# ai-forever/Kandinsky-5

Measured on AMD Instinct MI355X. Metric: DiT denoising steps/sec (2B Lite, 5s 768x512 latent), higher is better.
Workload: dtype bf16

## Files before the change

include/k5.h:

```cpp
#ifndef K5_H
#define K5_H
#include <stdint.h>
#ifdef __cplusplus
extern "C" {
#endif

typedef enum {
  K5_OK = 0, K5_ERR_ARG = 1, K5_ERR_ALIGN = 2, K5_ERR_HIP = 3, K5_ERR_STATE = 4, K5_ERR_KEY = 5,
  K5_ERR_UNSUPPORTED = 6
} k5_status;
typedef enum { K5_F32 = 0, K5_BF16 = 1, K5_F16 = 2 } k5_dtype;
typedef enum { K5_EPI_BIAS = 0, K5_EPI_BIAS_M = 1, K5_EPI_GELU = 2, K5_EPI_GATE = 3, K5_EPI_F32 = 4  } k5_epilogue;

#define K5_ABI_VERSION 11
int k5_abi_version(void);
const char* k5_last_error(void);


int k5_gemm_bf16(const void* A, const void* W, const float* bias, void* C, int M, int N, int K, int lda,
                 int ldw, int ldc, int epilogue, const void* resid, int ldr, const float* gate, void* stream);
int k5_gemm_bf16_variant(const void* A, const void* W, const float* bias, void* C, int M, int N, int K, int lda, int ldw, int ldc,
                         int epilogue, const void* resid, int ldr, const float* gate, void* stream, int kernel, int token_tile);

int k5_gemm_bf16_f32out(const void* A, const void* W, float* C, int M, int N, int K, int lda, int ldw, int ldc,
// ... 37 lines not shown
                                          float* state, int flags, int late_pass, void* workspace, void* stream);
int k5_attention_bf16_prescaled_qnorm_pass(const void* Q, const void* Kc, const void* Vt, void* O, int H, int q_len, int kv_len, int ldq,
                                           int ldk, int ldvt, int ldo, const float* q_norm_w, const float* q_cos, const float* q_sin,
                                           int* head_flags, const float* kmax, int tile_off0, int tile_cnt, float* state, int flags,
                                           int late_pass, void* workspace, void* stream);
int k5_attention_bf16_prescaled_auto(const void* Q, const void* Kc, const void* Vt, void* O, int H, int q_len, int kv_len,
                                     int ldq, int ldk, int ldvt, int ldo, const int* head_flags, int variant, void* workspace,
                                     void* stream);
int64_t k5_attention_balance_size(int H, int q_len);
int k5_attention_bf16_balanced(const void* Q, const void* K, const void* Vt, void* O, int H, int q_len, int kv_len,
                               int ldq, int ldk, int ldvt, int ldo, float score_bound, void* workspace, void* stream);

int64_t k5_nabla_workspace_size(int H, int num_blocks);
int k5_nabla_select_bf16(const void* q, const void* k, int ldq, int ldk, int H, int N, int T, int Hb, int Wb, int wT,
                         int wH, int wW, float P, void* workspace, void* stream);
int k5_attention_nabla_bf16(const void* Q, const void* K, const void* Vt, void* O, int H, int N, int ldq, int ldk,
                            int ldvt, int ldo, float score_bound, const void* workspace, void* stream);
int k5_nabla_mask_u8(const void* workspace, int H, int num_blocks, void* out_u8, void* stream);
int k5_nabla_select_rect_bf16(const void* q, const void* k, int ldq, int ldk, int H, int Nq, int q_block0, int N, int T,
                              int Hb, int Wb, int wT, int wH, int wW, float P, void* workspace, void* stream);
int k5_attention_nabla_rect_bf16(const void* Q, const void* K, const void* Vt, void* O, int H, int Nq, int N, int ldq,
                                 int ldk, int ldvt, int ldo, float score_bound, const void* workspace, int vt_chunk_keys,
                                 int64_t vt_chunk_stride, void* stream);
int k5_nabla_select_rect_local_bf16(const void* q, const void* k, int ldq, int ldk, int H, int Nq, int q_block0, int N, int T, int Hb,
                                    int Wb, int wT, int wH, int wW, float P, void* workspace, int local_block0, int local_blocks,
                                    void* stream);
int k5_attention_nabla_rect_prescaled_pass(const void* Q, const void* Kc, const void* Vt, void* O, int H, int Nq, int N, int ldq, int ldk,
                                           int ldvt, int ldo, const void* workspace, int vt_chunk_keys, int64_t vt_chunk_stride,
                                           int* head_flags, const float* kmax, int pass, float* state, void* stream);
int k5_nabla_mask_rect_u8(const void* workspace, int H, int q_blocks, int num_blocks, void* out_u8, void* stream);

int k5_attention_bf16_bounded(const void* Q, const void* K, const void* Vt, void* O, int H, int q_len,
                              int kv_len, int ldq, int ldk, int ldvt, int ldo, float score_bound, void* stream);

int k5_ln_modulate_bf16(const void* x, const float* scale, const float* shift, void* out, int rows, int D,
                        int ldx, int ldo, void* stream);
int k5_rmsnorm_rope_bf16(void* x, const float* weight, const float* cos_tab, const float* sin_tab, int rows,
                         int H, int ld, int heads_per_weight, int rope_heads, void* stream);
int k5_rmsnorm_rope_stats_bf16(void* x, const float* weight, const float* cos_tab, const float* sin_tab, int rows, int H,
                               int ld, int heads_per_weight, int rope_heads, float out_scale, int scale_from_head,
                               float* stats, void* stream);
int k5_gate_sum_bf16(const void* x, const void* y, const float* gate, void* out, int rows, int D, void* stream);
int k5_magcache_stats_bf16(const void* vis, const void* ori, const void* prev, void* res, double* sums, int rows, int D, void* stream);
int k5_gemv_f32(const float* x, const float* W, const float* b, float* y, int N, int K, int silu_in,
                const float* add, void* stream);
int k5_time_features_f32(float t, float* out, int D, void* stream);
int k5_ln_affine_bf16(const void* x, const float* w, const float* b, void* out_bf16, float* out_f32, int rows,
                      int D, void* stream);
int k5_rope_table_f32(float* cos_tab, float* sin_tab, const int32_t* pos_t, const int32_t* pos_h,
                      const int32_t* pos_w, int T, int H, int W, int n0, int n1, int n2, float s0, float s1,
                      float s2, const int32_t* tok_perm, void* stream);
int k5_patchify_bf16(const float* x, void* out, int T, int H, int W, int x_channels, int Cin_total, int Kpad,
                     const int32_t* tok_perm, void* stream);
int k5_patchify_cond_bf16(const float* x, const float* vcond, void* out, int T, int H, int W, int x_channels, int Cin_total,
                          int Kpad, const int32_t* tok_perm, void* stream);
int k5_unpatchify_bf16(const void* x, void* out, int T, int Hp, int Wp, int C, int ldx,
                       const int32_t* tok_perm, void* stream);
int k5_cfg_euler(float* img, const void* v_cond, const void* v_uncond, float w, float dt, int64_t n,
                 void* stream);

typedef struct k5_dit k5_dit;

typedef struct k5_dit_config {
  int in_visual_dim, in_text_dim, in_text_dim2, time_dim, out_visual_dim;
  int patch_size[3];
  int model_dim, ff_dim, num_text_blocks, num_visual_blocks;
// ... 139 lines not shown
```

kandinsky-5_amd/csrc/attn_fwd.hip:

```cpp
#include <stdlib.h>

#include <type_traits>
#include "k5_common.h"
#include "k5_kernels.h"

namespace {

constexpr int QB = 256;
constexpr int KB = 64;
constexpr int TILE = 64 * 128;

constexpr float K5_ATTN_EXP_LIMIT = 90.f;
constexpr float K5_ATTN_ROW_MIN = 3.2311743e-27f;
constexpr float K5_ATTN_ROWOFF_LIMIT = 190.f;
constexpr float K5_ATTN_ANCHOR_ADD = 20.f, K5_ATTN_ANCHOR_SPREAD = 1.4f, K5_ATTN_ANCHOR_EXTRA_MAX = 60.f;
inline float anchor_spread(int kv_total) {
  const float c = sqrtf(2.f * logf(512.f));
  return K5_ATTN_ANCHOR_SPREAD * (sqrtf(2.f * logf((float)(kv_total > 512 ? kv_total : 512))) - c) / c;
}
constexpr float K5_ATTN_ROW_MAX = 5.1922969e33f;
constexpr int K5_ANCHOR_TILES = 32;
#ifndef K5_ATTN_WAVE_ROWS_DEFAULT
#define K5_ATTN_WAVE_ROWS_DEFAULT 32
#endif
#ifndef K5_ATTN_PAIR
#define K5_ATTN_PAIR 1
#endif

struct AttnP {
  const bf16_t* Q; const bf16_t* K; const bf16_t* Vt; bf16_t* O;
  int H, q_len, kv_len, ldq, ldk, ldvt, ldo, nqb;
  float c;
  const int* sp_begin;
  const int* head_flags; int my_flag;
// ... 621 lines not shown
        float* st_o = state_o(qt); float* st_ml = state_ml(qt, g);
#pragma unroll
        for (int dt = 0; dt < 4; ++dt) *reinterpret_cast<f32x4*>(st_o + 256 * dt) = ot[dt][qt];
        st_ml[0] = BOUNDED ? 0.f : (fresh ? -1e30f : -nm[qt][0]);
        st_ml[1] = g == 0 ? lt[qt][0] : 0.f;
        if (BOUNDED && PRE && p.kmax && nm[qt][0] != 0.f && !((lt[qt][0] >= K5_ATTN_ROW_MIN || (anchored && !SPARSE)) && lt[qt][0] < K5_ATTN_ROW_MAX) && seen) {
          if (p.job_flags) const_cast<int*>(p.job_flags)[lid] = p.late_pass ? 2 : 1;
          else const_cast<int*>(p.head_flags)[h] = p.late_pass ? 2 : 0;
        }
      }
    return;
  }

#pragma unroll
  for (int qt = 0; qt < QT; ++qt) {
    const float l_tot = lt[qt][0];
    const float inv = l_tot > 0.f ? 1.0f / l_tot : 0.f;
    const int q = q0 + 16 * qt + l15;
    if (BOUNDED && PRE && p.kmax && q < p.q_len && nm[qt][0] != 0.f && !(l_tot >= K5_ATTN_ROW_MIN && l_tot < K5_ATTN_ROW_MAX)) {
      if (p.job_flags) const_cast<int*>(p.job_flags)[lid] = p.late_pass ? 2 : 1;
      else const_cast<int*>(p.head_flags)[h] = p.late_pass ? 2 : 0;
    }
    if (q < p.q_len) {
      bf16_t* op = p.O + (size_t)q * p.ldo + h * 64 + 4 * g;
#pragma unroll
      for (int dt = 0; dt < 4; ++dt) {
        u32x2 o = {pack_bf16x2(ot[dt][qt][0] * inv, ot[dt][qt][1] * inv), pack_bf16x2(ot[dt][qt][2] * inv, ot[dt][qt][3] * inv)};
        *reinterpret_cast<u32x2*>(op + 16 * dt) = o;
      }
    }
  }
}

template <bool BOUNDED, bool SPARSE, bool RANGE>
__global__ __launch_bounds__(512, 4) void attn_fwd32_kernel(AttnP p) {
  __shared__ __attribute__((aligned(16))) char smem[4 * TILE];
  char* sK = smem;
  char* sV = smem + 2 * TILE;
  const int tid = threadIdx.x, lane = tid & 63, wave = tid >> 6, hi = lane >> 5, l31 = lane & 31;
  const int gid = xcd_remap(blockIdx.x, gridDim.x);
  const int part = RANGE ? gid % p.splits : 0;
  const int lid = p.job0 + (RANGE ? gid / p.splits : gid);
  const int h = lid / p.nqb, qb = lid % p.nqb;
  const int q0 = qb * QB + wave * 32;

  bf16x8 qf[4];
  {
    const bf16_t* qp = p.Q + (size_t)min(q0 + l31, p.q_len - 1) * p.ldq + h * 64 + 8 * hi;
#pragma unroll
    for (int kk = 0; kk < 4; ++kk) qf[kk] = *reinterpret_cast<const bf16x8*>(qp + 16 * kk);
  }
  const int lrow = tid >> 3, lc = tid & 7;
  const bf16_t* kbase = p.K + h * 64 + 8 * lc;
  const bf16_t* vbase = p.Vt + (size_t)(h * 64 + lrow) * p.ldvt + 8 * lc;
  const int lds_off = lds_swz(lrow, lc);
  const int* sp_list = SPARSE ? p.sp_list + (size_t)(h * p.nqb + qb) * p.sp_stride : nullptr;
  const int Tall = SPARSE ? p.sp_cnt[h * p.nqb + qb] : p.tile_cnt;
  const int E0 = RANGE ? (int)(((long long)Tall * part) / p.splits) : 0;
  const int T = RANGE ? (int)(((long long)Tall * (part + 1)) / p.splits) : Tall;
  const int nfull = p.kv_len / KB;
  auto tile_of = [&](int e) -> int {
    if (SPARSE) return sp_list[e] & 0xffffff;
    if (!RANGE) return e;
    if (p.seg_len > 0) {
      int si = e / p.seg_len;
      const int j = e - si * p.seg_len;
// ... 313 lines not shown
      }
      const float extra = fminf(fmaxf(spread * (m - sm * inv_n), 0.f), K5_ATTN_ANCHOR_EXTRA_MAX);
      const int row = 64 * blk + 16 * qt + l15;
      if (g == 0 && row < q_len) out[(size_t)h * q_len + row] = ceilf(m + extra) + K5_ATTN_ANCHOR_ADD;
    }
  }
}

}


size_t k5_attention_state_bytes(int H, int q_len) { return (size_t)H * ((q_len + QB - 1) / QB) * QB * (64 + 8) * sizeof(float); }

constexpr int K5_ATTN_MAX_SPLITS = 6;
size_t k5_attention_balance_bytes(int H, int q_len) {
  return (size_t)K5_ATTN_MAX_SPLITS * k5_attention_state_bytes(H, q_len) + (size_t)H * ((q_len + 63) / 64 + 1) * sizeof(int);
}
namespace {
inline int* attn_job_flags(float* ws, int H, int q_len) { return reinterpret_cast<int*>(reinterpret_cast<char*>(ws) + (size_t)K5_ATTN_MAX_SPLITS * k5_attention_state_bytes(H, q_len)); }
inline size_t attn_job_flags_bytes(int H, int q_len) { return (size_t)H * ((q_len + 63) / 64 + 1) * sizeof(int); }
}

namespace {
int g_attn_slots = 0;
int attn_slots() {
  if (!g_attn_slots) {
    int dev = 0; hipDeviceProp_t prop;
    if (hipGetDevice(&dev) != hipSuccess || hipGetDeviceProperties(&prop, dev) != hipSuccess) return 512;
    g_attn_slots = 2 * (prop.multiProcessorCount > 0 ? prop.multiProcessorCount : 256);
  }
  static const bool pipe = getenv("K5_ATTN_WAVE_ROWS") && atoi(getenv("K5_ATTN_WAVE_ROWS")) > 100;
  return pipe ? g_attn_slots / 2 : g_attn_slots;
}
}

int k5_launch_attn_pref_update(float* balance_ws, int H, int q_len, int group_rows, int* prefer_online, hipStream_t stream, unsigned int* leave_sig) {
  if (!balance_ws || !prefer_online || H <= 0 || q_len <= 0) return K5_ERR_ARG;
  const int nqb = (q_len + 64 * group_rows - 1) / (64 * group_rows);
  hipLaunchKernelGGL(attn_pref_update_kernel, dim3(H), dim3(64), 0, stream, attn_job_flags(balance_ws, H, q_len), nqb, H, prefer_online, leave_sig);
  return hipGetLastError() == hipSuccess ? K5_OK : K5_ERR_HIP;
}

int k5_launch_attn_flags(float* qstat, float* kstat, int nk, int kstride, int H, int force_online, int* flags,
                         unsigned long long* counters, hipStream_t stream, float* kmax_out, const int* prefer_online, float* rstat, float* krad_out,
                         int nq, int qstride, bool anchored, unsigned int* leave_sig) {
  if ((rstat == nullptr) != (krad_out == nullptr) || (rstat && !kmax_out) || nq < 1) return K5_ERR_ARG;
  if (!qstat || !kstat || !flags || H <= 0 || nk <= 0) return K5_ERR_ARG;
  hipLaunchKernelGGL(attn_flags_kernel, dim3((H + 63) / 64), dim3(64), 0, stream, qstat, kstat, nk, kstride, H,
                     kmax_out ? K5_ATTN_ROWOFF_LIMIT : K5_ATTN_EXP_LIMIT, force_online, flags, counters, kmax_out, kmax_out ? prefer_online : nullptr,
                     rstat, krad_out, nq, qstride, anchored ? 1 : 0, leave_sig);
  return hipGetLastError() == hipSuccess ? K5_OK : K5_ERR_HIP;
}

int k5_launch_attn_row_anchor(const void* Q, const void* Kc, int H, int q_len, int kv_len, int ldq, int ldk, int key0, int kv_total,
                              const float* kmax, float* out, hipStream_t stream) {
  if (!Q || !Kc || !kmax || !out || H <= 0 || q_len <= 0 || kv_len < KB || (kv_len % KB) || (ldq & 7) || (ldk & 7)) return K5_ERR_ARG;
  hipLaunchKernelGGL(attn_row_anchor_kernel, dim3((q_len + 1023) / 1024, H), dim3(512), 0, stream, (const bf16_t*)Q, (const bf16_t*)Kc, q_len, kv_len,
                     ldq, ldk, key0, anchor_spread(kv_total > kv_len ? kv_total : kv_len), kmax, out);
  return hipGetLastError() == hipSuccess ? K5_OK : K5_ERR_HIP;
}

int k5_launch_attention_bf16_range(const void* Q, const void* K, const void* Vt, void* O, int H, int q_len,
                                   int kv_len, int ldq, int ldk, int ldvt, int ldo, float score_bound,
                                   int vt_chunk_keys, long long vt_chunk_stride, int tile_off0, int tile_cnt, int tile_skip_at,
                                   int tile_skip_n, float* state, int flags, hipStream_t stream, float* ws, bool k_prescaled,
                                   const int* head_flags, int variant, const K5TileSegments* seg, const float* kmax, int late_pass,
                                   const K5QueryNorm* qn, const K5KeyCentre* kc) {
// ... 20 lines not shown
  }
  p.q_norm_w = qn ? qn->w : nullptr; p.q_cos = qn ? qn->cos : nullptr; p.q_sin = qn ? qn->sin : nullptr;
  p.variant_counters = qn ? qn->counters : nullptr;
  if (p.q_norm_w) {
    if (k_prescaled) {
      if (!p.q_cos || !p.q_sin || (kmax && !head_flags)) return K5_ERR_ARG;
    } else if (!(score_bound > 0.f && score_bound * p.c <= K5_ATTN_EXP_LIMIT)) {
      return K5_ERR_UNSUPPORTED;
    }
  }
  p.vt_chunk_keys = vt_chunk_keys; p.vt_chunk_stride = vt_chunk_stride;
  const dim3 block(512);
  const bool bounded = score_bound > 0.f && score_bound * p.c <= K5_ATTN_EXP_LIMIT;
  p.sp_list = nullptr; p.sp_cnt = nullptr; p.sp_stride = 0;
  const int total_tiles = (kv_len + KB - 1) / KB;
  if (tile_cnt < 0) tile_cnt = total_tiles - tile_off0;
  p.seg_len = 0; p.seg_stride = 0; p.seg_skip = 0x7fffffff;
  if (seg && seg->len > 0) {
    if (tile_off0 < 0 || tile_cnt <= 0 || seg->stride < seg->len || seg->skip < 0) return K5_ERR_ARG;
    int si = (tile_cnt - 1) / seg->len;
    const int j = (tile_cnt - 1) - si * seg->len;
    if (si >= seg->skip) ++si;
    if ((long long)tile_off0 + (long long)si * seg->stride + j >= total_tiles) return K5_ERR_ARG;
    p.seg_len = seg->len; p.seg_stride = seg->stride; p.seg_skip = seg->skip;
    tile_skip_at = 0x7fffffff; tile_skip_n = 0;
  } else if (tile_off0 < 0 || tile_skip_n < 0 || tile_off0 + tile_cnt + (tile_skip_at < total_tiles ? tile_skip_n : 0) > total_tiles) return K5_ERR_ARG;
  if ((flags & 3) && !state) return K5_ERR_ARG;
  p.tile_off0 = tile_off0; p.tile_cnt = tile_cnt; p.tile_skip_at = tile_skip_at; p.tile_skip_n = tile_skip_n;
  p.state = state; p.flags = flags;
  p.job0 = 0; p.splits = 1; p.split_state = nullptr; p.split_stride = 0;
  const bool range = tile_off0 != 0 || tile_cnt != total_tiles || (flags & 3) || p.seg_len > 0;
  if (k_prescaled && (kv_len % KB)) return K5_ERR_ARG;
  if ((head_flags || variant != K5_ATTN_AUTO) && !k_prescaled) return K5_ERR_ARG;
  const bool run_fixed = head_flags ? variant == K5_ATTN_AUTO : (variant == K5_ATTN_AUTO && bounded);
  const bool run_online = head_flags ? true : !run_fixed;
  auto launch = [&](int njobs, bool use_range) {
    const dim3 grid(njobs);
    if (k_prescaled) {
      p.head_flags = (run_fixed && run_online) ? head_flags : nullptr;
      if (p.q_norm_w) {
        if (run_fixed) { p.my_flag = 1; hipLaunchKernelGGL((attn_fwd_kernel<true, false, true, true, true>), grid, block, 0, stream, p); }
        if (run_online) { p.my_flag = 0; hipLaunchKernelGGL((attn_fwd_kernel<false, false, true, true, true>), grid, block, 0, stream, p); }
      } else {
        static const int wave_rows = getenv("K5_ATTN_WAVE_ROWS") ? atoi(getenv("K5_ATTN_WAVE_ROWS")) : K5_ATTN_WAVE_ROWS_DEFAULT;
        if (run_fixed) {
          p.my_flag = 1;
          if (wave_rows == 64) hipLaunchKernelGGL((attn_fwd_kernel<true, false, true, true, false, 4, 4>), grid, dim3(256), 0, stream, p);
          else if (wave_rows == 132) {
            static bool attr = false;
            if (!attr) {
              if (hipFuncSetAttribute((const void*)attn_fwd_kernel<true, false, true, true, false, 4, 2, true>, hipFuncAttributeMaxDynamicSharedMemorySize, 12 * TILE) != hipSuccess) return;
              attr = true;
            }
            hipLaunchKernelGGL((attn_fwd_kernel<true, false, true, true, false, 4, 2, true>), grid, block, 12 * TILE, stream, p);
          }
          else if (wave_rows == 164) {
            static bool attr = false;
            if (!attr) {
              if (hipFuncSetAttribute((const void*)attn_fwd_kernel<true, false, true, true, false, 4, 4, true>, hipFuncAttributeMaxDynamicSharedMemorySize, 12 * TILE) != hipSuccess) return;
              attr = true;
            }
            hipLaunchKernelGGL((attn_fwd_kernel<true, false, true, true, false, 4, 4, true>), grid, dim3(256), 12 * TILE, stream, p);
          }
          else hipLaunchKernelGGL((attn_fwd_kernel<true, false, true, true>), grid, block, 0, stream, p);
        }
        if (run_online) { p.my_flag = 0; hipLaunchKernelGGL((attn_fwd_kernel<false, false, true, true>), grid, block, 0, stream, p); }
// ... 131 lines not shown
```

kandinsky-5_amd/csrc/engine.hip:

```cpp
#include <math.h>
#include <stdarg.h>
#include <stdio.h>
#include <string.h>

#include <map>
#include <string>
#include <vector>

#include <dlfcn.h>
#include <pthread.h>
#include <rccl/rccl.h>

#include "k5_common.h"
#include "k5_kernels.h"
#include "ipc_comm.h"

static thread_local char g_err[1024] = "";
void k5_set_error(const char* fmt, ...) {
  va_list ap;
  va_start(ap, fmt);
  vsnprintf(g_err, sizeof(g_err), fmt, ap);
  va_end(ap);
}
extern "C" const char* k5_last_error(void) { return g_err; }
// ... 2267 lines not shown
  K5CHK(ipc_open(d->comm, shm_name, rank, world));
  K5CHK(comm_common_init(d, rank, world));
  d->sp_autotune = false;
  return K5_OK;
}
extern "C" int k5_dit_cfg_pair_init_ipc(k5_dit* d, const char* shm_name, int branch) {
  g_err[0] = 0;
  if (!d || !shm_name || branch < 0 || branch > 1) return K5_ERR_ARG;
  K5CHK(ipc_open(d->pair, shm_name, branch, 2));
  return pair_common_init(d, branch);
}

extern "C" int k5_dit_set_option(k5_dit* d, const char* name, int value) {
  g_err[0] = 0;
  if (!d || !name) return K5_ERR_ARG;
  if (!strcmp(name, "attn_mode")) {
    if (value != K5_ATTN_AUTO && value != K5_ATTN_ONLINE) { k5_set_error("attn_mode must be 0 or 1"); return K5_ERR_ARG; }
    d->attn_mode = value; return K5_OK;
  }
  if (!strcmp(name, "sp_pass1_tiles")) { if (value < 0) return K5_ERR_ARG; d->sp_pass1_tiles = value; return K5_OK; }
  if (!strcmp(name, "sp_mode")) { if (value < 0 || value > 2) return K5_ERR_ARG; d->sp_mode = value; d->sp_user_set |= 1; return K5_OK; }
  if (!strcmp(name, "sp_autotune")) { d->sp_autotune = value != 0; if (value > 1) d->sp_tuned = false; return K5_OK; }
  if (!strcmp(name, "attn_row_offsets")) { d->row_offsets = value != 0; return K5_OK; }
  if (!strcmp(name, "attn_anchor")) { d->anchor = value != 0; return K5_OK; }
  if (!strcmp(name, "attn_pref_reset")) return reset_attn_pref(d, nullptr, true);
  if (!strcmp(name, "cross_kv_batched")) { if (value != 0 && value != 1) return K5_ERR_ARG; d->cross_kv_batched = value; return K5_OK; }
  if (!strcmp(name, "nabla_fuse_means")) { if (value < 0 || value > 2) return K5_ERR_ARG; d->nabla_fuse_means = value; return K5_OK; }
  if (!strcmp(name, "fp8_fuse_ln")) { if (value != 0 && value != 1) return K5_ERR_ARG; d->fp8_fuse_ln = value; return K5_OK; }
  if (!strcmp(name, "nabla_pair_frames")) { if (value != 0 && value != 1) return K5_ERR_ARG; d->nabla_pair_frames = value; return K5_OK; }
  if (!strcmp(name, "nabla_group_rows")) { if (value != 0 && value != 1 && value != 2 && value != 4) return K5_ERR_ARG; d->nabla_group_rows = value; return K5_OK; }
  if (!strcmp(name, "sp_nabla_passes")) { if (value < 1 || value > 2) return K5_ERR_ARG; d->sp_nabla_passes = value; d->sp_user_set |= 4; return K5_OK; }
  if (!strcmp(name, "attn_fuse_qnorm")) { if (value < 0 || value > 2) return K5_ERR_ARG; d->fuse_qnorm = value; return K5_OK; }
  if (!strcmp(name, "attn_fuse_qnorm_auto")) { if (value != 0 && value != 1) return K5_ERR_ARG; d->fuse_qnorm_auto = value; return K5_OK; }
  if (!strcmp(name, "sp_slices")) {
    if (value < 1 || value > 4) return K5_ERR_ARG;
    if (value > 1 && d->comm.comm && !d->comm.can_exchange()) { k5_set_error("sp_slices > 1 needs ncclSend / ncclRecv / ncclGroup* in the RCCL library"); return K5_ERR_STATE; }
    d->sp_slices = value; d->sp_user_set |= 2; return K5_OK;
  }
  if (!strcmp(name, "emulate_world")) {
    if (!d->comm.active() || d->comm.world != 1 || value < 1) { k5_set_error("emulate_world needs a world = 1 communicator"); return K5_ERR_STATE; }
    d->sp_world = value; d->emulated = value > 1;
    if (d->emulated) fprintf(stderr, "libk5: emulate_world=%d — timing-only layout, the results of this handle are garbage\n", value);
    return K5_OK;
  }
  k5_set_error("unknown option %s", name);
  return K5_ERR_ARG;
}
extern "C" int k5_dit_get_option(k5_dit* d, const char* name, int* value) {
  if (!d || !name || !value) return K5_ERR_ARG;
  if (!strcmp(name, "attn_mode")) *value = d->attn_mode;
  else if (!strcmp(name, "sp_pass1_tiles")) *value = d->sp_pass1_tiles;
  else if (!strcmp(name, "sp_mode")) *value = d->sp_mode;
  else if (!strcmp(name, "sp_mode_used")) *value = d->sp_mode_used;
  else if (!strcmp(name, "sp_slices")) *value = d->sp_slices;
  else if (!strcmp(name, "attn_row_offsets")) *value = d->row_offsets ? 1 : 0;
  else if (!strcmp(name, "attn_anchor")) *value = d->anchor ? 1 : 0;
  else if (!strcmp(name, "attn_fuse_qnorm")) *value = d->fuse_qnorm;
  else if (!strcmp(name, "attn_fuse_qnorm_auto")) *value = d->fuse_qnorm_auto;
  else if (!strcmp(name, "attn_fuse_qnorm_used")) *value = d->fuse_last;
  else if (!strcmp(name, "sp_nabla_passes")) *value = d->sp_nabla_passes;
  else if (!strcmp(name, "sp_autotune")) *value = d->sp_autotune ? 1 : 0;
  else if (!strcmp(name, "sp_tuned")) *value = d->sp_tuned ? 1 : 0;
  else if (!strcmp(name, "fp8_effective")) {
    int m = d->fp8_mask;
    if (d->comm.active()) { m &= ~4; if (sp_schedule(d, d->last_nabla) != 0) m &= ~2; }
    *value = m;
  }
  else if (!strcmp(name, "rccl_ranks")) {
    *value = 0;
    if (d->comm.comm && d->comm.CommCount) { int n = 0; *value = d->comm.CommCount(d->comm.comm, &n) == ncclSuccess ? n : -1; }
    else if (d->comm.active()) *value = -1;
  }
  else if (!strcmp(name, "ipc_ranks")) *value = d->comm.ipc ? d->comm.ipc->world : 0;
  else if (!strcmp(name, "ipc_pair_ranks")) *value = d->pair.ipc ? d->pair.ipc->world : 0;
  else if (!strcmp(name, "ipc_collectives")) *value = (int)((d->comm.ipc ? d->comm.ipc->collectives : 0) + (d->pair.ipc ? d->pair.ipc->collectives : 0));
  else if (!strcmp(name, "ipc_pulled_mb")) *value = (int)(((d->comm.ipc ? d->comm.ipc->bytes_pulled : 0) + (d->pair.ipc ? d->pair.ipc->bytes_pulled : 0)) >> 20);
  else if (!strcmp(name, "ipc_flags_finegrained")) *value = (d->comm.ipc && d->comm.ipc->flags_fine) ? 1 : 0;
  else if (!strcmp(name, "ipc_errors")) {
    *value = 0;
    for (Comm* c : {&d->comm, &d->pair}) if (c->ipc) { uint32_t w = 0; if (c->ipc->error_word(&w)) { k5_set_error("%s", c->ipc->err.c_str()); return K5_ERR_HIP; } if (w && !*value) *value = (int)w; }
  }
  else if (!strcmp(name, "nabla_group_rows")) *value = d->nabla_group_rows;
  else if (!strcmp(name, "nabla_pair_frames")) *value = d->nabla_pair_frames;
  else if (!strcmp(name, "fp8_fuse_ln")) *value = d->fp8_fuse_ln;
  else if (!strcmp(name, "nabla_fuse_means")) *value = d->nabla_fuse_means;
  else if (!strcmp(name, "cross_kv_batched")) *value = d->cross_kv_batched;
  else if (!strcmp(name, "emulate_world")) *value = d->emulated ? d->sp_world : 0;
  else if (!strcmp(name, "emulated")) *value = d->emulated ? 1 : 0;
  else { k5_set_error("unknown option %s", name); return K5_ERR_ARG; }
  return K5_OK;
}

extern "C" int k5_dit_attn_variant_counts(k5_dit* d, long long* fixed_heads, long long* online_heads, int reset) {
// ... 82 lines not shown
```

kandinsky-5_amd/csrc/k5_api.hip:

```cpp
#include "k5_kernels.h"

void k5_set_error(const char* fmt, ...);

static int ret(int st, const char* what) {
  if (st != K5_OK) {
    const hipError_t e = hipGetLastError();
    k5_set_error("%s: status %d (%s)", what, st, e == hipSuccess ? "argument/alignment" : hipGetErrorString(e));
  }
  return st;
}

extern "C" {

int k5_gemm_bf16(const void* A, const void* W, const float* bias, void* C, int M, int N, int K, int lda, int ldw,
                 int ldc, int epilogue, const void* resid, int ldr, const float* gate, void* stream) {
  return ret(k5_launch_gemm_bf16(A, W, bias, C, M, N, K, lda, ldw, ldc, epilogue, resid, ldr, gate, (hipStream_t)stream),
             "k5_gemm_bf16");
}

int k5_gemm_bf16_variant(const void* A, const void* W, const float* bias, void* C, int M, int N, int K, int lda, int ldw,
                         int ldc, int epilogue, const void* resid, int ldr, const float* gate, void* stream, int kernel, int token_tile) {
  if (token_tile != 0 && token_tile != 128 && token_tile != 192 && token_tile != 256) return ret(K5_ERR_ARG, "k5_gemm_bf16_variant");
  return ret(k5_launch_gemm_bf16(A, W, bias, C, M, N, K, lda, ldw, ldc, epilogue, resid, ldr, gate, (hipStream_t)stream, kernel, token_tile / 32),
             "k5_gemm_bf16_variant");
// ... 170 lines not shown
             "k5_attention_nabla_rect_bf16");
}

int k5_nabla_select_rect_local_bf16(const void* q, const void* k, int ldq, int ldk, int H, int Nq, int q_block0, int N, int T, int Hb,
                                    int Wb, int wT, int wH, int wW, float P, void* workspace, int local_block0, int local_blocks,
                                    void* stream) {
  return ret(k5_launch_nabla_select_rect(q, k, ldq, ldk, H, Nq, q_block0, N, T, Hb, Wb, wT, wH, wW, P, workspace,
                                         (hipStream_t)stream, local_block0, local_blocks), "k5_nabla_select_rect_local_bf16");
}
int k5_attention_nabla_rect_prescaled_pass(const void* Q, const void* Kc, const void* Vt, void* O, int H, int Nq, int N, int ldq, int ldk,
                                           int ldvt, int ldo, const void* workspace, int vt_chunk_keys, int64_t vt_chunk_stride,
                                           int* head_flags, const float* kmax, int pass, float* state, void* stream) {
  if (!workspace || N <= 0 || (N % 64) || pass < 0 || pass > 2 || (pass && !state) || !head_flags || !kmax)
    return ret(K5_ERR_ARG, "k5_attention_nabla_rect_prescaled_pass");
  const int *list, *cnt, *cnt_local;
  if (Nq <= 0 || (Nq % 64)) return ret(K5_ERR_ARG, "k5_attention_nabla_rect_prescaled_pass");
  k5_nabla_workspace_views(const_cast<void*>(workspace), H, N / 64, nullptr, nullptr, &list, &cnt, &cnt_local, Nq / 64);
  const K5SparsePass p1{nullptr, state, 2, 1}, p2{cnt_local, state, 1, 2};
  return ret(k5_launch_attention_bf16_sparse(Q, Kc, Vt, O, H, Nq, N, ldq, ldk, ldvt, ldo, 0.f, list, pass == 1 ? cnt_local : cnt, N / 64,
                                             vt_chunk_keys, (long long)vt_chunk_stride, (hipStream_t)stream, true, head_flags, K5_ATTN_AUTO,
                                             kmax, pass == 0 ? nullptr : (pass == 1 ? &p1 : &p2)),
             "k5_attention_nabla_rect_prescaled_pass");
}

int k5_nabla_mask_rect_u8(const void* workspace, int H, int q_blocks, int num_blocks, void* out_u8, void* stream) {
  return ret(k5_launch_nabla_mask_u8(workspace, H, q_blocks, num_blocks, out_u8, (hipStream_t)stream), "k5_nabla_mask_rect_u8");
}

int k5_attention_bf16_bounded(const void* Q, const void* K, const void* Vt, void* O, int H, int q_len, int kv_len,
                              int ldq, int ldk, int ldvt, int ldo, float score_bound, void* stream) {
  return ret(k5_launch_attention_bf16_bounded(Q, K, Vt, O, H, q_len, kv_len, ldq, ldk, ldvt, ldo, score_bound,
                                              (hipStream_t)stream), "k5_attention_bf16_bounded");
}

int k5_ln_modulate_bf16(const void* x, const float* scale, const float* shift, void* out, int rows, int D, int ldx,
                        int ldo, void* stream) {
  return ret(k5_launch_ln_modulate(x, scale, shift, out, rows, D, ldx, ldo, (hipStream_t)stream), "k5_ln_modulate_bf16");
}

int k5_rmsnorm_rope_bf16(void* x, const float* weight, const float* cos_tab, const float* sin_tab, int rows, int H,
                         int ld, int heads_per_weight, int rope_heads, void* stream) {
  const int32_t hc[2] = {heads_per_weight, rope_heads};
  return ret(k5_launch_rmsnorm_rope(x, weight, cos_tab, sin_tab, rows, H, ld, hc, (hipStream_t)stream),
             "k5_rmsnorm_rope_bf16");
}

int k5_rmsnorm_rope_stats_bf16(void* x, const float* weight, const float* cos_tab, const float* sin_tab, int rows, int H, int ld,
                               int heads_per_weight, int rope_heads, float out_scale, int scale_from_head, float* stats, void* stream) {
  const int32_t hc[2] = {heads_per_weight, rope_heads};
  static float* ws = nullptr; static size_t ws_bytes = 0;
  const size_t need = k5_rmsnorm_stats_workspace_bytes(H);
  if (stats && need > ws_bytes) {
    if (ws) (void)hipFree(ws);
    ws = nullptr; ws_bytes = 0;
    if (hipMalloc((void**)&ws, need) != hipSuccess) return ret(K5_ERR_HIP, "k5_rmsnorm_rope_stats_bf16");
    ws_bytes = need;
  }
  return ret(k5_launch_rmsnorm_rope(x, weight, cos_tab, sin_tab, rows, H, ld, hc, (hipStream_t)stream, out_scale, scale_from_head,
                                    nullptr, 0, stats, ws), "k5_rmsnorm_rope_stats_bf16");
}

int k5_rmsnorm_rope_centre_bf16(void* x, const float* weight, const float* cos_tab, const float* sin_tab, int rows, int H, int ld,
                                int heads_per_weight, int rope_heads, float out_scale, int scale_from_head, float* stats, float* centre, void* stream) {
  if (!stats || !centre || scale_from_head < 0 || scale_from_head >= H) return ret(K5_ERR_ARG, "k5_rmsnorm_rope_centre_bf16");
  const int32_t hc[2] = {heads_per_weight, rope_heads};
  static float* ws = nullptr; static size_t ws_bytes = 0;
// ... 108 lines not shown
```

kandinsky-5_amd/csrc/k5_kernels.h:

```cpp
#pragma once
#include <hip/hip_runtime.h>
#include <stdint.h>

#include "k5.h"

int k5_launch_gemm_bf16(const void* A, const void* W, const float* bias, void* C, int M, int N, int K,
                        int lda, int ldw, int ldc, int epi, const void* resid, int ldr,
                        const float* gate, hipStream_t stream,
                        int force_kernel = 0,
                        int force_mt = 0);

int k5_launch_attention_bf16_bounded(const void* Q, const void* K, const void* Vt, void* O, int H, int q_len,
                                     int kv_len, int ldq, int ldk, int ldvt, int ldo, float score_bound,
                                     hipStream_t stream);

int k5_launch_attention_bf16_chunked(const void* Q, const void* K, const void* Vt, void* O, int H, int q_len,
                                     int kv_len, int ldq, int ldk, int ldvt, int ldo, float score_bound,
                                     int vt_chunk_keys, long long vt_chunk_stride, hipStream_t stream);

size_t k5_attention_state_bytes(int H, int q_len);
struct K5TileSegments { int len, stride, skip; };
struct K5SparsePass { const int* begin; float* state; int flags; int late_pass; };
struct K5QueryNorm { const float* w; const float* cos; const float* sin; unsigned long long* counters; };
struct K5KeyCentre { const float* centre; const float* radius; const float* row_anchor = nullptr; };
int k5_launch_attention_bf16_range(const void* Q, const void* K, const void* Vt, void* O, int H, int q_len,
                                   int kv_len, int ldq, int ldk, int ldvt, int ldo, float score_bound,
                                   int vt_chunk_keys, long long vt_chunk_stride, int tile_off0, int tile_cnt, int tile_skip_at,
                                   int tile_skip_n, float* state, int flags, hipStream_t stream, float* balance_ws = nullptr, bool k_prescaled = false,
                                   const int* head_flags = nullptr, int variant = 0, const K5TileSegments* segments = nullptr,
                                   const float* row_offset_kmax = nullptr, int late_pass = 0,
                                   const K5QueryNorm* query_norm = nullptr,
                                   const K5KeyCentre* key_centre = nullptr);
size_t k5_attention_balance_bytes(int H, int q_len);
enum { K5_ATTN_AUTO = 0, K5_ATTN_ONLINE = 1 };
int k5_launch_attn_flags(float* qstat, float* kstat, int nk, int kstride, int H, int force_online, int* flags,
                         unsigned long long* counters, hipStream_t stream, float* kmax_out = nullptr, const int* prefer_online = nullptr,
                         float* rstat = nullptr, float* krad_out = nullptr,
                         int nq = 1, int qstride = 0,
                         bool anchored = false,
                         unsigned int* leave_sig = nullptr);
int k5_launch_attn_row_anchor(const void* Q, const void* Kc, int H, int q_len, int kv_len, int ldq, int ldk, int key0, int kv_total,
                              const float* kmax, float* out, hipStream_t stream);
int k5_launch_attn_pref_update(float* balance_ws, int H, int q_len, int group_rows, int* prefer_online, hipStream_t stream,
                               unsigned int* leave_sig = nullptr);

int k5_launch_gemm_fp8(const void* A8, const void* W8, const float* w_scale, void* C, int M, int N, int K, int lda, int ldw, int ldc,
                       int epi, const void* resid, int ldr, const float* gate, hipStream_t stream, const float* bias = nullptr, int scale_m = 0);
int k5_launch_quant_rows_fp8(const void* x, void* out, float* scale, int rows, int K, int ldx, int ldo, hipStream_t stream);

size_t k5_nabla_workspace_bytes(int H, int nb, int nqb = 0, int list_rows = 0);
int k5_launch_nabla_select(const void* q, const void* k, int ldq, int ldk, int H, int N, int T, int Hb, int Wb, int wT, int wH,
                           int wW, float P, void* workspace, hipStream_t s);
void k5_nabla_workspace_views(void* workspace, int H, int nb, const unsigned long long** bits, const int** kv_nb, const int** list,
                              const int** cnt, const int** cnt_local = nullptr, int nqb = 0);
int k5_launch_nabla_select_rect(const void* q, const void* k, int ldq, int ldk, int H, int Nq, int q_block0, int N, int T, int Hb,
                                int Wb, int wT, int wH, int wW, float P, void* workspace, hipStream_t s,
                                int local_block0 = 0, int local_blocks = 0,
                                int group_rows = 4,
                                int pair_stride = 0);
int k5_launch_nabla_block_means(const void* x, int ld, int H, int nblocks, int stride_blocks, void* out, hipStream_t s);
void k5_nabla_workspace_means(void* workspace, int H, int nb, void** qa, void** ka);
int k5_launch_nabla_key_means_from_slots(const void* gathered, int H, int nb, int slot_blocks, void* workspace, hipStream_t s);
int k5_launch_nabla_mask_u8(const void* workspace, int H, int nqb, int nb, void* out, hipStream_t s);
int k5_launch_nabla_count(const void* workspace, int H, int nqb, int nb, unsigned long long* acc, hipStream_t s);
int k5_launch_nabla_count_lists(const void* workspace, int H, int nqb, int nb, int group_rows, unsigned long long* acc, hipStream_t s);
int k5_launch_attention_bf16_sparse(const void* Q, const void* K, const void* Vt, void* O, int H, int q_len, int kv_len, int ldq,
// ... 73 lines not shown
```

kandinsky-5_amd/kandinsky/_engine.py:

```python
from __future__ import annotations

import ctypes as C
import os
from typing import Optional

import torch

_HERE = os.path.dirname(os.path.abspath(__file__))
LIB_PATH = os.environ.get("K5_LIB", os.path.join(os.path.dirname(_HERE), "lib", "libk5.so"))

K5_OK = 0
ABI_VERSION = 11
K5_F32, K5_BF16, K5_F16 = 0, 1, 2
EPI_BIAS, EPI_BIAS_M, EPI_GELU, EPI_GATE = 0, 1, 2, 3

_DT = {torch.float32: K5_F32, torch.bfloat16: K5_BF16, torch.float16: K5_F16}


class DitConfig(C.Structure):
    _fields_ = [("in_visual_dim", C.c_int), ("in_text_dim", C.c_int), ("in_text_dim2", C.c_int),
                ("time_dim", C.c_int), ("out_visual_dim", C.c_int), ("patch_size", C.c_int * 3),
                ("model_dim", C.c_int), ("ff_dim", C.c_int), ("num_text_blocks", C.c_int),
                ("num_visual_blocks", C.c_int), ("axes_dims", C.c_int * 3), ("visual_cond", C.c_int)]

# ... 57 lines not shown
    "k5_attention_row_anchor": (_I, [_P, _P, _I, _I, _I, _I, _I, _I, _I, _P, _P, _P]),
    "k5_attention_bf16_prescaled_rows_anchored": (_I, [_P, _P, _P, _P, _I, _I, _I, _I, _I, _I, _I, _P, _P, _P, _P, _P, _P, _P]),
    "k5_rmsnorm_rope_stats_bf16": (_I, [_P, _P, _P, _P, _I, _I, _I, _I, _I, _F, _I, _P, _P]),
    "k5_loopback_create": (_I, [_I, C.POINTER(_P)]),
    "k5_loopback_destroy": (None, [_P]),
    "k5_dit_comm_init_loopback": (_I, [_P, _P, _I]),
    "k5_dit_cfg_pair_init": (_I, [_P, C.c_char_p, _I, _P]),
    "k5_dit_cfg_pair_init_loopback": (_I, [_P, _P, _I]),
    "k5_dit_comm_init_ipc": (_I, [_P, C.c_char_p, _I, _I]),
    "k5_dit_cfg_pair_init_ipc": (_I, [_P, C.c_char_p, _I]),
    "k5_dit_cfg_branch": (_I, [_P]),
    "k5_dit_set_option": (_I, [_P, C.c_char_p, _I]),
    "k5_dit_get_option": (_I, [_P, C.c_char_p, C.POINTER(_I)]),
    "k5_dit_sp_schedule": (_I, [_P, C.c_char_p, _I]),
    "k5_sp_pick_schedule": (_I, [C.POINTER(C.c_float), _I, _I, C.POINTER(_I), C.POINTER(C.c_float)]),
    "k5_sp_plan_2d": (_I, [_I, _I, _I, _I, _I, C.POINTER(_I), C.POINTER(C.c_longlong)]),
    "k5_dit_attn_variant_counts": (_I, [_P, C.POINTER(C.c_longlong), C.POINTER(C.c_longlong), _I]),
    "k5_dit_nabla_block_counts": (_I, [_P, C.POINTER(C.c_longlong), C.POINTER(C.c_longlong)]),
    "k5_dit_set_nabla_tap": (_I, [_P, _P, C.c_longlong]),
    "k5_dit_nabla_tap_count": (_I, [_P, C.POINTER(C.c_longlong)]),
    "k5_dit_nabla_executed_blocks": (_I, [_P, C.POINTER(C.c_longlong)]),
    "k5_attention_balance_size": (_I64, [_I, _I]),
    "k5_attention_bf16_balanced": (_I, [_P, _P, _P, _P, _I, _I, _I, _I, _I, _I, _I, _F, _P, _P]),
    "k5_nabla_workspace_size": (_I64, [_I, _I]),
    "k5_nabla_select_bf16": (_I, [_P, _P, _I, _I, _I, _I, _I, _I, _I, _I, _I, _I, _F, _P, _P]),
    "k5_attention_nabla_bf16": (_I, [_P, _P, _P, _P, _I, _I, _I, _I, _I, _I, _F, _P, _P]),
    "k5_nabla_mask_u8": (_I, [_P, _I, _I, _P, _P]),
    "k5_nabla_select_rect_bf16": (_I, [_P, _P, _I, _I, _I, _I, _I, _I, _I, _I, _I, _I, _I, _I, _F, _P, _P]),
    "k5_attention_nabla_rect_bf16": (_I, [_P, _P, _P, _P, _I, _I, _I, _I, _I, _I, _I, _F, _P, _I, _I64, _P]),
    "k5_nabla_select_rect_local_bf16": (_I, [_P, _P, _I, _I, _I, _I, _I, _I, _I, _I, _I, _I, _I, _I, _F, _P, _I, _I, _P]),
    "k5_attention_nabla_rect_prescaled_pass": (_I, [_P, _P, _P, _P, _I, _I, _I, _I, _I, _I, _I, _P, _I, _I64, _P, _P, _I, _P, _P]),
    "k5_nabla_mask_rect_u8": (_I, [_P, _I, _I, _I, _P, _P]),
    "k5_attention_bf16_bounded": (_I, [_P, _P, _P, _P, _I, _I, _I, _I, _I, _I, _I, _F, _P]),
    "k5_ln_modulate_bf16": (_I, [_P, _P, _P, _P, _I, _I, _I, _I, _P]),
    "k5_rmsnorm_rope_bf16": (_I, [_P, _P, _P, _P, _I, _I, _I, _I, _I, _P]),
    "k5_gate_sum_bf16": (_I, [_P, _P, _P, _P, _I, _I, _P]),
    "k5_magcache_stats_bf16": (_I, [_P, _P, _P, _P, _P, _I, _I, _P]),
    "k5_gemv_f32": (_I, [_P, _P, _P, _P, _I, _I, _I, _P, _P]),
    "k5_time_features_f32": (_I, [_F, _P, _I, _P]),
    "k5_ln_affine_bf16": (_I, [_P, _P, _P, _P, _P, _I, _I, _P]),
    "k5_rope_table_f32": (_I, [_P, _P, _P, _P, _P, _I, _I, _I, _I, _I, _I, _F, _F, _F, _P, _P]),
    "k5_patchify_bf16": (_I, [_P, _P, _I, _I, _I, _I, _I, _I, _P, _P]),
    "k5_patchify_cond_bf16": (_I, [_P, _P, _P, _I, _I, _I, _I, _I, _I, _P, _P]),
    "k5_unpatchify_bf16": (_I, [_P, _P, _I, _I, _I, _I, _I, _P, _P]),
    "k5_cfg_euler": (_I, [_P, _P, _P, _F, _F, _I64, _P]),
    "k5_dit_create": (_I, [C.POINTER(DitConfig), C.POINTER(_P)]),
    "k5_dit_destroy": (None, [_P]),
    "k5_dit_load_tensor": (_I, [_P, C.c_char_p, _P, _I, C.POINTER(_I64), _I]),
    "k5_dit_finalize": (_I, [_P]),
    "k5_dit_missing_keys": (_I, [_P]),
    "k5_dit_forward": (_I, [_P, C.POINTER(ForwardArgs), _P, _P]),
    "k5_sample": (_I, [_P, C.POINTER(SampleArgs), _P]),
    "k5_sample_cond": (_I, [_P, C.POINTER(SampleArgs), _P, _P]),
    "k5_sample_many": (_I, [_P, C.POINTER(SampleManyArgs), _P]),
    "k5_dit_forward_many": (_I, [_P, C.POINTER(ForwardArgs), _I, C.POINTER(TextCond), _P, _P]),
    "k5_comm_unique_id": (_I, [C.c_char_p, _P]),
    "k5_dit_comm_init": (_I, [_P, C.c_char_p, _I, _I, _P]),
    "k5_conv3d_bf16": (_I, [_P, _P, _P, _P, _I, _I, _I, _I, _I, _I, _I, _I, _P, _I, _P]),
    "k5_conv3d_strided_bf16": (_I, [_P, _P, _P, _P, _I, _I, _I, _I, _I, _I, _I, _I, _P]),
    "k5_groupnorm_workspace_size": (_I64, [_I, _I]),
    "k5_groupnorm_bf16": (_I, [_P, _P, _P, _P, _I, _I, _I, _F, _I, _P, _P]),
    "k5_conv3d_stats_size": (_I64, [_I, _I]),
    "k5_conv3d_bf16_stats": (_I, [_P, _P, _P, _P, _I, _I, _I, _I, _I, _I, _I, _I, _P, _I, _P, _P]),
    "k5_groupnorm_bf16_quads": (_I, [_P, _P, _P, _P, _I, _I, _I, _F, _I, _P, _P, _P]),
    "k5_vae_path_counts": (_I, [_P, C.POINTER(C.c_longlong), _I]),
    "k5_vae_create": (_I, [C.POINTER(VaeConfig), C.POINTER(_P)]),
# ... 214 lines not shown
```

Measured before the change: 1.893.

## Add short-KV attention kernel keeping all keys/values resident in LDS

Adds a specialised attention kernel for bounded attention with at most four key tiles (kv_len ≤ 256). It loads all K/V tiles into shared memory once per block and loops over several query tiles per block, skipping the online-softmax and anchor machinery. The kernel can also apply a fused query RMS-norm. This targets short cross-attention such as visual-to-text, where per-launch overhead and repeated K/V loads dominate. The cost is doubled LDS per block (which may lower occupancy) and a second code path whose numerics could differ from the general bounded kernel.

```diff
diff --git a/include/k5.h b/include/k5.h
--- a/include/k5.h
+++ b/include/k5.h
@@ -93,6 +93,10 @@
 
 int k5_attention_bf16_bounded(const void* Q, const void* K, const void* Vt, void* O, int H, int q_len,
                               int kv_len, int ldq, int ldk, int ldvt, int ldo, float score_bound, void* stream);
+int k5_attention_bf16_bounded_qnorm(const void* Q, const void* K, const void* Vt, void* O, int H, int q_len, int kv_len, int ldq, int ldk,
+                                    int ldvt, int ldo, float score_bound, const float* q_norm_w, void* stream);
+int k5_attention_short_set(int on);
+int64_t k5_attention_short_launches(void);
 
 int k5_ln_modulate_bf16(const void* x, const float* scale, const float* shift, void* out, int rows, int D,
                         int ldx, int ldo, void* stream);
diff --git a/kandinsky-5_amd/csrc/attn_fwd.hip b/kandinsky-5_amd/csrc/attn_fwd.hip
--- a/kandinsky-5_amd/csrc/attn_fwd.hip
+++ b/kandinsky-5_amd/csrc/attn_fwd.hip
@@ -1,5 +1,6 @@
 #include <stdlib.h>
 
+#include <atomic>
 #include <type_traits>
 #include "k5_common.h"
 #include "k5_kernels.h"
@@ -687,6 +688,170 @@
   }
 }
 
+struct AttnShortP {
+  const bf16_t* Q; const bf16_t* K; const bf16_t* Vt; bf16_t* O;
+  const float* q_norm_w;
+  int q_len, kv_len, ldq, ldk, ldvt, ldo, nqb, spw;
+  float c;
+};
+
+__global__ __launch_bounds__(512, 4) void attn_short_kernel(AttnShortP p) {
+  constexpr int QT = 2;
+  __shared__ __attribute__((aligned(16))) char smem[8 * TILE];
+  char* sK = smem;
+  char* sV = smem + 4 * TILE;
+  const int tid = threadIdx.x, lane = tid & 63, wave = tid >> 6, g = lane >> 4, l15 = lane & 15;
+  const int h = blockIdx.x / p.spw, slot = blockIdx.x - h * p.spw;
+  const int t_begin = (int)(((long long)p.nqb * slot) / p.spw), t_end = (int)(((long long)p.nqb * (slot + 1)) / p.spw);
+  if (t_begin >= t_end) return;
+  const int T = p.kv_len / KB;
+  {
+    const int lrow = tid >> 3, lc = tid & 7;
+    const int wave_u = __builtin_amdgcn_readfirstlane(wave);
+    const char* Kb = reinterpret_cast<const char*>(p.K);
+    const char* Vb = reinterpret_cast<const char*>(p.Vt);
+    const uint32_t kstride = (uint32_t)p.ldk * 2u;
+    const uint32_t klane = (uint32_t)(h * 64 + 8 * (lc ^ (((lrow >> 1) & 1) | (((lrow >> 3) & 3) << 1)))) * 2u;
+    const uint32_t vlane = ((uint32_t)(h * 64 + lrow) * (uint32_t)p.ldvt + 8u * (lc ^ ((lrow >> 1) & 7))) * 2u;
+    typedef __attribute__((address_space(3))) void lds_void_t;
+    typedef const __attribute__((address_space(1))) void gbl_void_t;
+#pragma unroll
+    for (int t = 0; t < 4; ++t) {
+      if (t < T) {
+        __builtin_amdgcn_global_load_lds((gbl_void_t*)(Kb + ((uint32_t)(t * KB + lrow) * kstride + klane)), (lds_void_t*)(sK + t * TILE + wave_u * 1024), 16, 0, 0);
+        __builtin_amdgcn_global_load_lds((gbl_void_t*)(Vb + 2 * (t * KB) + vlane), (lds_void_t*)(sV + t * TILE + wave_u * 1024), 16, 0, 0);
+      }
+    }
+  }
+  auto load_q = [&](int tile, bf16x8 (&q)[QT][2]) {
+#pragma unroll
+    for (int qt = 0; qt < QT; ++qt) {
+      const bf16_t* qp = p.Q + (size_t)min(tile * QB + wave * 32 + 16 * qt + l15, p.q_len - 1) * p.ldq + h * 64 + 8 * g;
+#pragma unroll
+      for (int ks = 0; ks < 2; ++ks) q[qt][ks] = *reinterpret_cast<const bf16x8*>(qp + 32 * ks);
+    }
+  };
+  bf16x8 qn[QT][2];
+  load_q(t_begin, qn);
+  __syncthreads();
+  const int krow = 8 * (l15 >> 2) + (l15 & 3);
+  const bf16x8 onesf = __builtin_bit_cast(bf16x8, u32x4{0x3f803f80u, 0x3f803f80u, 0x3f803f80u, 0x3f803f80u});
+  const float c = p.c;
+  for (int tile = t_begin; tile < t_end; ++tile) {
+    bf16x8 qf[QT][2];
+#pragma unroll
+    for (int qt = 0; qt < QT; ++qt)
+#pragma unroll
+      for (int ks = 0; ks < 2; ++ks) qf[qt][ks] = qn[qt][ks];
+    if (p.q_norm_w) {
+      f32x4 wa[2], wb[2];
+#pragma unroll
+      for (int ks = 0; ks < 2; ++ks) {
+        wa[ks] = *reinterpret_cast<const f32x4*>(p.q_norm_w + 32 * ks + 8 * g);
+        wb[ks] = *reinterpret_cast<const f32x4*>(p.q_norm_w + 32 * ks + 8 * g + 4);
+      }
+#pragma unroll
+      for (int qt = 0; qt < QT; ++qt) {
+        float v[16], ss = 0.f;
+#pragma unroll
+        for (int ks = 0; ks < 2; ++ks) {
+          const u32x4 w4 = __builtin_bit_cast(u32x4, qf[qt][ks]);
+#pragma unroll
+          for (int j = 0; j < 4; ++j) {
+            v[8 * ks + 2 * j] = __uint_as_float(w4[j] << 16);
+            v[8 * ks + 2 * j + 1] = __uint_as_float(w4[j] & 0xffff0000u);
+            ss += v[8 * ks + 2 * j] * v[8 * ks + 2 * j] + v[8 * ks + 2 * j + 1] * v[8 * ks + 2 * j + 1];
+          }
+        }
+        {
+          const auto s16 = __builtin_amdgcn_permlane16_swap(__float_as_uint(ss), __float_as_uint(ss), false, false);
+          ss = __uint_as_float(s16[0]) + __uint_as_float(s16[1]);
+          const auto s32 = __builtin_amdgcn_permlane32_swap(__float_as_uint(ss), __float_as_uint(ss), false, false);
+          ss = __uint_as_float(s32[0]) + __uint_as_float(s32[1]);
+        }
+        const float rs = rsqrtf(ss * (1.0f / 64.0f) + 1.1920928955078125e-07f);
+#pragma unroll
+        for (int ks = 0; ks < 2; ++ks) {
+          float y[8];
+#pragma unroll
+          for (int j = 0; j < 8; ++j) y[j] = __fmul_rn(__fmul_rn(v[8 * ks + j], rs), j < 4 ? wa[ks][j] : wb[ks][j - 4]);
+          const u32x4 pk = {pack_bf16x2(y[0], y[1]), pack_bf16x2(y[2], y[3]), pack_bf16x2(y[4], y[5]), pack_bf16x2(y[6], y[7])};
+          qf[qt][ks] = __builtin_bit_cast(bf16x8, pk);
+        }
+      }
+    }
+    if (tile + 1 < t_end) load_q(tile + 1, qn);
+    f32x4 ot[4][QT], lt[QT];
+#pragma unroll
+    for (int qt = 0; qt < QT; ++qt) {
+      lt[qt] = f32x4{0.f, 0.f, 0.f, 0.f};
+#pragma unroll
+      for (int dt = 0; dt < 4; ++dt) ot[dt][qt] = f32x4{0.f, 0.f, 0.f, 0.f};
+    }
+#pragma unroll
+    for (int e = 0; e < 4; ++e) {
+      if (e < T) {
+        const char* cK = sK + e * TILE;
+        const char* cV = sV + e * TILE;
+        const f32x4 zero4 = f32x4{0.f, 0.f, 0.f, 0.f};
+#pragma unroll
+        for (int ks2 = 0; ks2 < 2; ++ks2) {
+          f32x4 st[2][QT];
+#pragma unroll
+          for (int k2 = 0; k2 < 2; ++k2) {
+            const bf16x8 kf = *reinterpret_cast<const bf16x8*>(cK + lds_swz_k(krow + 32 * ks2 + 4 * k2, g));
+#pragma unroll
+            for (int qt = 0; qt < QT; ++qt) st[k2][qt] = mfma16(kf, qf[qt][0], zero4);
+          }
+#pragma unroll
+          for (int k2 = 0; k2 < 2; ++k2) {
+            const bf16x8 kf = *reinterpret_cast<const bf16x8*>(cK + lds_swz_k(krow + 32 * ks2 + 4 * k2, 4 + g));
+#pragma unroll
+            for (int qt = 0; qt < QT; ++qt) st[k2][qt] = mfma16(kf, qf[qt][1], st[k2][qt]);
+          }
+          bf16x8 pf[QT];
+#pragma unroll
+          for (int qt = 0; qt < QT; ++qt) {
+            float ev[8];
+#pragma unroll
+            for (int j = 0; j < 8; ++j) ev[j] = __builtin_amdgcn_exp2f(st[j >> 2][qt][j & 3] * c);
+            const u32x4 pk = {pack_bf16x2(ev[0], ev[1]), pack_bf16x2(ev[2], ev[3]), pack_bf16x2(ev[4], ev[5]), pack_bf16x2(ev[6], ev[7])};
+            pf[qt] = __builtin_bit_cast(bf16x8, pk);
+            lt[qt] = mfma16(onesf, pf[qt], lt[qt]);
+          }
+#pragma unroll
+          for (int dt = 0; dt < 4; ++dt) {
+            const bf16x8 vf = *reinterpret_cast<const bf16x8*>(cV + lds_swz(16 * dt + l15, 4 * ks2 + g));
+#pragma unroll
+            for (int qt = 0; qt < QT; ++qt) ot[dt][qt] = mfma16(vf, pf[qt], ot[dt][qt]);
+          }
+        }
+      }
+    }
+#pragma unroll
+    for (int qt = 0; qt < QT; ++qt) {
+      const float l_tot = lt[qt][0];
+      const float inv = l_tot > 0.f ? 1.0f / l_tot : 0.f;
+      const int q = tile * QB + wave * 32 + 16 * qt + l15;
+      uint32_t pk[4][2];
+#pragma unroll
+      for (int dt = 0; dt < 4; ++dt) {
+        pk[dt][0] = pack_bf16x2(ot[dt][qt][0] * inv, ot[dt][qt][1] * inv);
+        pk[dt][1] = pack_bf16x2(ot[dt][qt][2] * inv, ot[dt][qt][3] * inv);
+      }
+#pragma unroll
+      for (int dp = 0; dp < 2; ++dp) {
+        const auto s0 = __builtin_amdgcn_permlane16_swap(pk[2 * dp][0], pk[2 * dp + 1][0], false, false);
+        const auto s1 = __builtin_amdgcn_permlane16_swap(pk[2 * dp][1], pk[2 * dp + 1][1], false, false);
+        if (q < p.q_len) {
+          const u32x4 o = {s0[0], s1[0], s0[1], s1[1]};
+          *reinterpret_cast<u32x4*>(p.O + (size_t)q * p.ldo + h * 64 + 16 * (2 * dp + (g & 1)) + 8 * (g >> 1)) = o;
+        }
+      }
+    }
+  }
+}
+
 template <bool BOUNDED, bool SPARSE, bool RANGE>
 __global__ __launch_bounds__(512, 4) void attn_fwd32_kernel(AttnP p) {
   __shared__ __attribute__((aligned(16))) char smem[4 * TILE];
@@ -1066,7 +1231,14 @@
   static const bool pipe = getenv("K5_ATTN_WAVE_ROWS") && atoi(getenv("K5_ATTN_WAVE_ROWS")) > 100;
   return pipe ? g_attn_slots / 2 : g_attn_slots;
 }
-}
+int attn_short_slots() { attn_slots(); return g_attn_slots ? g_attn_slots : 512; }
+int g_attn_short = 1;
+std::atomic<long long> g_attn_short_launches{0};
+}
+
+void k5_attn_short_enable(int on) { g_attn_short = on != 0; }
+int k5_attn_short_enabled() { return g_attn_short; }
+long long k5_attn_short_count() { return g_attn_short_launches.load(std::memory_order_relaxed); }
 
 int k5_launch_attn_pref_update(float* balance_ws, int H, int q_len, int group_rows, int* prefer_online, hipStream_t stream, unsigned int* leave_sig) {
   if (!balance_ws || !prefer_online || H <= 0 || q_len <= 0) return K5_ERR_ARG;
@@ -1153,6 +1325,18 @@
   const bool range = tile_off0 != 0 || tile_cnt != total_tiles || (flags & 3) || p.seg_len > 0;
   if (k_prescaled && (kv_len % KB)) return K5_ERR_ARG;
   if ((head_flags || variant != K5_ATTN_AUTO) && !k_prescaled) return K5_ERR_ARG;
+  if (g_attn_short && !k_prescaled && bounded && !range && kv_len <= 4 * KB && (kv_len % KB) == 0 && vt_chunk_keys == 0 &&
+      ldq >= H * 64 && ldk >= H * 64 && ldo >= H * 64 && ldvt >= kv_len && (ldo & 7) == 0 &&
+      ((uintptr_t)Q & 15) == 0 && ((uintptr_t)K & 15) == 0 && ((uintptr_t)Vt & 15) == 0 && ((uintptr_t)O & 15) == 0) {
+    AttnShortP sp;
+    sp.Q = p.Q; sp.K = p.K; sp.Vt = p.Vt; sp.O = p.O; sp.q_norm_w = p.q_norm_w;
+    sp.q_len = q_len; sp.kv_len = kv_len; sp.ldq = ldq; sp.ldk = ldk; sp.ldvt = ldvt; sp.ldo = ldo; sp.nqb = p.nqb; sp.c = p.c;
+    const int per_head = attn_short_slots() / H;
+    sp.spw = per_head < 1 ? 1 : (per_head > p.nqb ? p.nqb : per_head);
+    hipLaunchKernelGGL(attn_short_kernel, dim3(H * sp.spw), block, 0, stream, sp);
+    g_attn_short_launches.fetch_add(1, std::memory_order_relaxed);
+    return hipGetLastError() == hipSuccess ? K5_OK : K5_ERR_HIP;
+  }
   const bool run_fixed = head_flags ? variant == K5_ATTN_AUTO : (variant == K5_ATTN_AUTO && bounded);
   const bool run_online = head_flags ? true : !run_fixed;
   auto launch = [&](int njobs, bool use_range) {
diff --git a/kandinsky-5_amd/csrc/engine.hip b/kandinsky-5_amd/csrc/engine.hip
--- a/kandinsky-5_amd/csrc/engine.hip
+++ b/kandinsky-5_amd/csrc/engine.hip
@@ -2323,6 +2323,7 @@
   if (!strcmp(name, "sp_nabla_passes")) { if (value < 1 || value > 2) return K5_ERR_ARG; d->sp_nabla_passes = value; d->sp_user_set |= 4; return K5_OK; }
   if (!strcmp(name, "attn_fuse_qnorm")) { if (value < 0 || value > 2) return K5_ERR_ARG; d->fuse_qnorm = value; return K5_OK; }
   if (!strcmp(name, "attn_fuse_qnorm_auto")) { if (value != 0 && value != 1) return K5_ERR_ARG; d->fuse_qnorm_auto = value; return K5_OK; }
+  if (!strcmp(name, "attn_short")) { if (value != 0 && value != 1) return K5_ERR_ARG; k5_attn_short_enable(value); return K5_OK; }
   if (!strcmp(name, "sp_slices")) {
     if (value < 1 || value > 4) return K5_ERR_ARG;
     if (value > 1 && d->comm.comm && !d->comm.can_exchange()) { k5_set_error("sp_slices > 1 needs ncclSend / ncclRecv / ncclGroup* in the RCCL library"); return K5_ERR_STATE; }
@@ -2350,6 +2351,8 @@
   else if (!strcmp(name, "attn_fuse_qnorm_auto")) *value = d->fuse_qnorm_auto;
   else if (!strcmp(name, "attn_fuse_qnorm_used")) *value = d->fuse_last;
   else if (!strcmp(name, "sp_nabla_passes")) *value = d->sp_nabla_passes;
+  else if (!strcmp(name, "attn_short")) *value = k5_attn_short_enabled();
+  else if (!strcmp(name, "attn_short_launches")) *value = (int)(k5_attn_short_count() & 0x7fffffff);
   else if (!strcmp(name, "sp_autotune")) *value = d->sp_autotune ? 1 : 0;
   else if (!strcmp(name, "sp_tuned")) *value = d->sp_tuned ? 1 : 0;
   else if (!strcmp(name, "fp8_effective")) {
diff --git a/kandinsky-5_amd/csrc/k5_api.hip b/kandinsky-5_amd/csrc/k5_api.hip
--- a/kandinsky-5_amd/csrc/k5_api.hip
+++ b/kandinsky-5_amd/csrc/k5_api.hip
@@ -226,6 +226,18 @@
   return ret(k5_launch_attention_bf16_bounded(Q, K, Vt, O, H, q_len, kv_len, ldq, ldk, ldvt, ldo, score_bound,
                                               (hipStream_t)stream), "k5_attention_bf16_bounded");
 }
+
+int k5_attention_bf16_bounded_qnorm(const void* Q, const void* K, const void* Vt, void* O, int H, int q_len, int kv_len, int ldq, int ldk,
+                                    int ldvt, int ldo, float score_bound, const float* q_norm_w, void* stream) {
+  if (!q_norm_w) return ret(K5_ERR_ARG, "k5_attention_bf16_bounded_qnorm");
+  const K5QueryNorm qn{q_norm_w, nullptr, nullptr, nullptr};
+  return ret(k5_launch_attention_bf16_range(Q, K, Vt, O, H, q_len, kv_len, ldq, ldk, ldvt, ldo, score_bound, 0, 0, 0, -1, 0x7fffffff, 0,
+                                            nullptr, 0, (hipStream_t)stream, nullptr, false, nullptr, K5_ATTN_AUTO, nullptr, nullptr, 0, &qn),
+             "k5_attention_bf16_bounded_qnorm");
+}
+
+int k5_attention_short_set(int on) { const int was = k5_attn_short_enabled(); k5_attn_short_enable(on); return was; }
+int64_t k5_attention_short_launches(void) { return (int64_t)k5_attn_short_count(); }
 
 int k5_ln_modulate_bf16(const void* x, const float* scale, const float* shift, void* out, int rows, int D, int ldx,
                         int ldo, void* stream) {
diff --git a/kandinsky-5_amd/csrc/k5_kernels.h b/kandinsky-5_amd/csrc/k5_kernels.h
--- a/kandinsky-5_amd/csrc/k5_kernels.h
+++ b/kandinsky-5_amd/csrc/k5_kernels.h
@@ -32,6 +32,9 @@
                                    const K5QueryNorm* query_norm = nullptr,
                                    const K5KeyCentre* key_centre = nullptr);
 size_t k5_attention_balance_bytes(int H, int q_len);
+void k5_attn_short_enable(int on);
+int k5_attn_short_enabled();
+long long k5_attn_short_count();
 enum { K5_ATTN_AUTO = 0, K5_ATTN_ONLINE = 1 };
 int k5_launch_attn_flags(float* qstat, float* kstat, int nk, int kstride, int H, int force_online, int* flags,
                          unsigned long long* counters, hipStream_t stream, float* kmax_out = nullptr, const int* prefer_online = nullptr,
diff --git a/kandinsky-5_amd/kandinsky/_engine.py b/kandinsky-5_amd/kandinsky/_engine.py
--- a/kandinsky-5_amd/kandinsky/_engine.py
+++ b/kandinsky-5_amd/kandinsky/_engine.py
@@ -113,6 +113,9 @@
     "k5_attention_nabla_rect_prescaled_pass": (_I, [_P, _P, _P, _P, _I, _I, _I, _I, _I, _I, _I, _P, _I, _I64, _P, _P, _I, _P, _P]),
     "k5_nabla_mask_rect_u8": (_I, [_P, _I, _I, _I, _P, _P]),
     "k5_attention_bf16_bounded": (_I, [_P, _P, _P, _P, _I, _I, _I, _I, _I, _I, _I, _F, _P]),
+    "k5_attention_bf16_bounded_qnorm": (_I, [_P, _P, _P, _P, _I, _I, _I, _I, _I, _I, _I, _F, _P, _P]),
+    "k5_attention_short_set": (_I, [_I]),
+    "k5_attention_short_launches": (_I64, []),
     "k5_ln_modulate_bf16": (_I, [_P, _P, _P, _P, _I, _I, _I, _I, _P]),
     "k5_rmsnorm_rope_bf16": (_I, [_P, _P, _P, _P, _I, _I, _I, _I, _I, _P]),
     "k5_gate_sum_bf16": (_I, [_P, _P, _P, _P, _I, _I, _P]),
```

New measurement: 1.898, median of 2. About the same (+0.3%).
